# AndersTrier/reed-solomon-simd

Hardware: AMD Instinct MI355X
Metric: GiB/s (original+recovery) encode & decode, device-resident, 1024:1024×1024B (higher is better)
Workload: dtype u8; 1 GPU; encode 1024:1024 x 1024 B, device-resident (rs_encode_device); original_count=1024, recovery_count=1024, parallelism=replicas x1 (independent stripes)

## Files before the change

__graft_entry__.py:

```python
import os
import subprocess
import sys

ROOT = os.path.dirname(os.path.abspath(__file__))
PKG = os.path.join(ROOT, "reed-solomon-simd_amd")
LIB = os.path.join(PKG, "lib", "librs_mi355x.so")
SOURCES = ["csrc/rs_kernels.hip", "csrc/rs_mono.hip", "csrc/rs_repair.hip", "csrc/rs_lane.hip", "csrc/rs_chunks.hip", "csrc/rs_eval.hip", "csrc/rs_update.hip", "csrc/rs_verify.hip", "csrc/rs_codec.cpp", "csrc/gf_tables.cpp"]
HEADERS = ["csrc/rs_device.hpp", "csrc/rs_gf.hpp", "csrc/gf_tables.hpp"]
INCLUDES = {"csrc/rs_repair.hip": ["csrc/rs_mono.hip"], "csrc/rs_verify.hip": ["csrc/rs_mono.hip"]}
HIPCC = os.environ.get("HIPCC", "/opt/rocm/bin/hipcc")
FLAGS = ["--offload-arch=gfx950", "-O3", "-std=c++17", "-fPIC", "-Wall"]
SOURCE_FLAGS = {"csrc/rs_mono.hip": ["-mllvm", "-amdgpu-kernarg-preload-count=14"]}


def _obj(src):
    return os.path.join(PKG, "build", os.path.basename(src) + ".o")


def _stale(target, deps):
    if not os.path.exists(target):
        return True
    t = os.path.getmtime(target)
    return any(os.path.getmtime(d) > t for d in deps)


def build(force: bool = False) -> None:
    os.makedirs(os.path.join(PKG, "lib"), exist_ok=True)
    os.makedirs(os.path.join(PKG, "build"), exist_ok=True)
    hdrs = [os.path.join(PKG, h) for h in HEADERS] + [os.path.join(ROOT, "include", "rs_mi355x.h")]
    procs = []
    for src in SOURCES:
        path = os.path.join(PKG, src)
        deps = [path] + hdrs + [os.path.join(PKG, i) for i in INCLUDES.get(src, [])]
        if force or _stale(_obj(src), deps):
            procs.append(subprocess.Popen([HIPCC] + FLAGS + SOURCE_FLAGS.get(src, []) + ["-c", path, "-o", _obj(src)],
                                          cwd=PKG))
    for p in procs:
        if p.wait() != 0:
            raise RuntimeError(f"hipcc failed: {p.args}")
    objs = [_obj(s) for s in SOURCES]
    if force or procs or _stale(LIB, objs):
        subprocess.run([HIPCC, "--offload-arch=gfx950", "-shared", "-fPIC", "-o", LIB] + objs, check=True)
    ob_src = os.path.join(ROOT, "tools", "object_bench.cpp")
    ob = os.path.join(PKG, "lib", "rs_object_bench")
    if force or _stale(ob, [ob_src, LIB, os.path.join(ROOT, "include", "rs_mi355x.h")]):
        subprocess.run(["g++", "-O2", "-std=c++17", "-I", os.path.join(ROOT, "include"), ob_src, "-o", ob,
                        "-L", os.path.join(PKG, "lib"), "-lrs_mi355x", "-Wl,-rpath,$ORIGIN"], check=True)
    subprocess.run(["make", "-s", "-C", os.path.join(ROOT, "oracle")], check=True)
    sys.path.insert(0, PKG)
    import reed_solomon_simd


def smoke() -> None:
    import numpy as np
    import torch

    sys.path.insert(0, PKG)
    sys.path.insert(0, os.path.join(ROOT, "tests"))
    import oracle_lib as O
    import reed_solomon_simd as rs

# ... 25 lines not shown
```

reed-solomon-simd_amd/csrc/rs_mono.hip:

```cpp
#include <hip/hip_runtime.h>

#include <cstdio>
#include <type_traits>

#include "rs_device.hpp"
#include "rs_gf.hpp"

namespace rs {
namespace {

#ifdef RS_MONO_STAMPS
__device__ uint64_t g_mono_stamps[4096][24];
#ifdef RS_MONO_STAMP_WAIT
#define RS_MSTAMP_WAIT() asm volatile("s_waitcnt vmcnt(0) lgkmcnt(0)" ::: "memory")
#else
#define RS_MSTAMP_WAIT() asm volatile("" ::: "memory")
#endif
#define RS_MSTAMP(i)                                                                                 \
    do {                                                                                             \
        RS_MSTAMP_WAIT();                                                                            \
        if (threadIdx.x == blockDim.x - 64 && blockIdx.x + blockIdx.y * gridDim.x < 4096) g_mono_stamps[blockIdx.x + blockIdx.y * gridDim.x][i] = __builtin_amdgcn_s_memrealtime(); \
    } while (0)
#else
#define RS_MSTAMP(i)
#endif


struct Map {
    int reg[3];
    int lane[6];
    int wave[4];
};
enum : int { kOpLayer = 1, kOpXpose = 2, kOpRemap = 3 };
struct Op {
    int kind, bit, rs, ls;
};
constexpr int kMaxOps = 64;
struct Seq {
    int count = 0;
    Op ops[kMaxOps] = {};
    Map maps[kMaxOps + 1] = {};
};

constexpr int find_reg(const Map &m, int LR, int x) {
    for (int s = 0; s < LR; ++s)
        if (m.reg[s] == x) return s;
    return -1;
}
constexpr int find_lane(const Map &m, int x) {
    for (int j = 0; j < 6; ++j)
        if (m.lane[j] == x) return j;
    return -1;
}
constexpr int next_use(const int *bits, int nb, int from, int x) {
    for (int t = from; t < nb; ++t)
        if (bits[t] == x) return t;
    return 1 << 20;
}
constexpr void push(Seq &s, Op op, const Map &after) {
// ... 177 lines not shown
constexpr int pair_of(int i, int s) { return (i & ((1 << s) - 1)) | ((i >> (s + 1)) << s); }

__device__ __forceinline__ void load_tab(const uint32_t *img, int L, int x, uint32_t row, uint32_t (&t)[20]) {
    const uint32_t n = 1u << L;
    const uint32_t slot = n - (n >> x) + (row >> (x + 1));
#ifdef RS_MONO_FAKE_TABS
    for (int q = 0; q < 20; ++q) t[q] = slot * 0x01010101u + q;
    return;
#endif
    const uint4 *p = reinterpret_cast<const uint4 *>(img) + slot * 5u;
#pragma unroll
    for (int q = 0; q < 5; ++q) {
        const uint4 v = p[q];
        t[4 * q] = v.x, t[4 * q + 1] = v.y, t[4 * q + 2] = v.z, t[4 * q + 3] = v.w;
    }
}

struct GlobalTabs {
    const uint32_t *img;
    template <int L, int LR, typename S, int I, int PH>
    __device__ __forceinline__ void get(int x, uint32_t row, uint32_t (&t)[20]) const {
        load_tab(img, L, x, row, t);
    }
};


#ifndef RS_MONO_SPARE_BARRIERS
#define RS_MONO_SPARE_BARRIERS 0
#endif

template <int L, int LR, int SP = 0, int E = 4>
struct Stage {
    static constexpr bool SPLIT = Plan<L, LR, SP>::SPLIT;
    static constexpr int FLO = Plan<L, LR, SP>::FLO;
    static constexpr int TW = Fmt<E>::kTW;
    static constexpr uint32_t PC = Fmt<E>::kPC;
    static constexpr bool kBasis = E == 2 && RS_MONO_BASIS;
    static constexpr uint32_t LPC = kBasis ? 2 : PC;
    template <typename AT>
    static __device__ __forceinline__ void put(uint32_t *region, uint32_t q, const uint4 &v, AT at) {
        if constexpr (kBasis) {
            const uint32_t p0 = (q >> 1) * PC + (q & 1u) * 2u;
            uint4 a, b;
            basis2_expand(v, a, b);
            reinterpret_cast<uint4 *>(region)[at(p0)] = a;
            reinterpret_cast<uint4 *>(region)[at(p0 + 1)] = b;
        } else {
            reinterpret_cast<uint4 *>(region)[at(q)] = v;
        }
    }
    static constexpr int SW = 20;
    static constexpr uint32_t SPC = SW / 4;
    static constexpr bool kGray = E == 2;
    static __device__ __forceinline__ uint32_t sg(uint32_t g) { return kGray ? g ^ ((g >> 1) & 15u) : g; }
    static __device__ __forceinline__ uint32_t sq(uint32_t t, uint32_t k) {
        if constexpr (!kGray) return t;
        const uint32_t y = (1u << k) - t;
        const uint32_t mask = y <= 1u ? 0u : (1u << (31 - __builtin_clz(y - 1u))) - 1u;
        return t ^ (((t & mask) >> 1) & 15u);
    }
    template <typename F>
    static __device__ __forceinline__ uint32_t at(uint32_t q, F f) {
        const uint32_t t = q / PC;
        return f(t) * SPC + (q - t * PC);
    }
    static __device__ __forceinline__ uint32_t at1(uint32_t q) {
        return at(q, [](uint32_t t) { return sq(t, uint32_t(IW - B0)); });
    }
    static __device__ __forceinline__ uint32_t at0(uint32_t q) { return at(q, [](uint32_t t) { return sg(t); }); }
    static __device__ __forceinline__ uint32_t atS(uint32_t q) {
        return at(q, [](uint32_t t) {
            if (t < kShI) return sq(t, uint32_t(L - IW));
            if (t < kShI + kShF) return kShI + sq(t - kShI, uint32_t(L - FLO));
            return t;
        });
    }
    static constexpr int IW = LR + 6, WB = L - IW - (SPLIT ? 1 : 0);
    static constexpr uint32_t n = 1u << L, W = 1u << IW;
    static constexpr int NB3 = WB > 0 ? FLO : L;
#ifndef RS_MONO_B0_MIN_L
#define RS_MONO_B0_MIN_L 11
#endif
    static constexpr int B0 = L >= RS_MONO_B0_MIN_L ? 1 : 0;
    static constexpr uint32_t kPriv = B0 ? (W >> 1) : W - 1;
    static constexpr uint32_t kUp = (W >> B0) - 1;
    static constexpr uint32_t kP3 = (W >> B0) - (W >> NB3);
    static constexpr uint32_t kL0 = W >> 1;
    static constexpr uint32_t kShI = WB > 0 ? (n >> IW) - 1 : 0;
    static constexpr uint32_t kShF = WB > 0 ? (n >> FLO) - 1 : 0;
    static constexpr uint32_t kShared = kShI + kShF;
    static constexpr uint32_t kWaves = 1u << (L - LR - 6);
    static constexpr uint32_t plane_words = (E == 4 ? 2 : 1) * n;
    static constexpr uint32_t words = plane_words + (kShared + kWaves * kPriv) * SW;
#ifdef RS_MONO_ENC_DERIVE3
    static constexpr bool kDerive3 = true;
#else
    static constexpr bool kDerive3 = false;
#endif
    static constexpr uint32_t kD = kDerive3 ? NB3 : 0;
    static constexpr uint32_t words_enc = words + kD * SW;
    static constexpr bool kPlane2 = RS_MONO_SPARE_BARRIERS && WB > 0 && (words_enc + plane_words) * 4 <= 160 * 1024;
    static constexpr uint32_t words_enc2 = words_enc + (kPlane2 ? plane_words : 0);
    static constexpr uint32_t words_dec = words + n;
    static constexpr uint32_t words_split = words_dec + (SPLIT ? plane_words : 0);
    static_assert(L > 11 || (words_enc2 * 4 <= 160 * 1024 && words_split * 4 <= 160 * 1024), "column kernel: LDS per workgroup");
};

template <int L, int LR, int SPLIT = 0, int E = 4>
struct LdsTabs {
    using G = Stage<L, LR, SPLIT, E>;
    const uint32_t *priv, *shared, *img_i, *img_f;
    template <int, int, typename S, int I, int PH>
    __device__ __forceinline__ void get(int x, uint32_t row, uint32_t (&t)[Fmt<E>::kTW]) const {
#ifdef RS_MONO_FAKE_TABS
        const uint32_t *fb = tab<0, 0, S, I, PH>(x, row);
        for (int q = 0; q < G::TW; ++q) t[q] = q + uint32_t(reinterpret_cast<uintptr_t>(fb));
        return;
#endif
        read(tab<0, 0, S, I, PH>(x, row), t);
    }
    static __device__ __forceinline__ void read(const uint32_t *tb, uint32_t (&t)[Fmt<E>::kTW]) {
        const uint4 *p = reinterpret_cast<const uint4 *>(tb);
#pragma unroll
        for (int q = 0; q < int(G::PC); ++q) {
            const uint4 v = p[q];
            t[4 * q] = v.x, t[4 * q + 1] = v.y, t[4 * q + 2] = v.z, t[4 * q + 3] = v.w;
        }
    }
    template <int, int, typename S, int I, int PH>
    __device__ __forceinline__ const uint32_t *tab(int x, uint32_t row) const {
        uint32_t slot;
        const uint32_t *base;
        if constexpr ((PH == 1 || PH == 3) && G::B0 == 1 && S::v.ops[I].bit == 0) {
            slot = G::sg((row & (G::W - 1)) >> 1);
            base = priv;
        } else if constexpr (PH == 1 || PH == 3) {
            slot = (G::W >> G::B0) - (G::W >> x) + G::sg((row & (G::W - 1)) >> (x + 1));
            base = priv;
        } else if constexpr (PH == 2) {
            slot = (G::n >> G::IW) - (G::n >> x) + G::sg(row >> (x + 1));
            base = shared;
        } else {
            slot = G::kShI + (G::n >> G::FLO) - (G::n >> x) + G::sg(row >> (x + 1));
// ... 1018 lines not shown
        walsh_lane<J, J>(x, lane);
    });
    walsh_reg<WB>(x);
    static_for<WB, 6>([&](auto jc) {
        constexpr int J = decltype(jc)::value;
        walsh_lane<J, J + 1>(x, lane);
    });
    RS_MSTAMP(20);
    eval_remap<L, false>(x, buf, lane, wave);
    static_for<6 - WB, 6>([&](auto jc) {
        constexpr int J = decltype(jc)::value;
        walsh_lane<J, J + WB + 1>(x, lane);
    });
    x[0] = walsh_fold(x[0]);
    x[1] = walsh_fold(x[1]);
    reinterpret_cast<uint2 *>(rinfo)[threadIdx.x] =
        uint2{x[0] | ((rbits & 1u) ? 0u : 0x10000u), x[1] | ((rbits & 2u) ? 0u : 0x10000u)};
    asm volatile("s_waitcnt lgkmcnt(0)" ::: "memory");
}

template <int L>
__device__ __forceinline__ void col_eval_poly(const MonoCore &A, uint32_t ebits, uint32_t rbits, const uint32_t &lwv,
                                              uint32_t *buf, uint32_t *rinfo) {
    if constexpr (kEvalRemap<L>) {
        col_eval_poly_remap<L>(A, ebits, rbits, lwv, buf, rinfo);
        return;
    }
    const uint32_t i0 = 2 * threadIdx.x;
    uint32_t x[2];
    static_for<0, 2>([&](auto kc) {
        constexpr int k = decltype(kc)::value;
        const uint32_t e = (ebits >> k) & 1u, i = i0 + k;
        x[k] = A.low_rate ? (i < A.end ? (e ? 0u : 65534u) : 0u) : e;
    });
    col_walsh<L, 0, 19>(x, buf);
    RS_MSTAMP(14);
    const uint32_t lw[2] = {lwv & 0xFFFFu, lwv >> 16};
    static_for<0, 2>([&](auto kc) {
        constexpr int k = decltype(kc)::value;
        const uint32_t p = x[k] * lw[k];
        uint32_t f = ev_add(p & 0xFFFFu, p >> 16);
        if (A.low_rate && i0 + k == 0) f = ev_add(f, A.lw0);
        x[k] = f;
    });
    col_walsh<L, kWalshRounds<L>, 20>(x, buf);
    reinterpret_cast<uint2 *>(rinfo)[threadIdx.x] =
        uint2{x[0] | ((rbits & 1u) ? 0u : 0x10000u), x[1] | ((rbits & 2u) ? 0u : 0x10000u)};
    asm volatile("s_waitcnt lgkmcnt(0)" ::: "memory");
}

template <int L, int LR, int SPLIT, int E>
__device__ __forceinline__ uint4 priv_piece(const uint32_t *img, uint32_t wave, uint32_t q) {
    using G = Stage<L, LR, SPLIT, E>;
    const uint32_t t = q / G::LPC, piece = q - t * G::LPC;
    const uint32_t y = (G::W >> G::B0) - t;
    const int b = G::IW - int(32 - __builtin_clz(y - 1));
    const uint32_t local = t - ((G::W >> G::B0) - (G::W >> b));
    const uint32_t slot = G::n - (G::n >> b) + wave * (G::W >> (b + 1)) + local;
    return reinterpret_cast<const uint4 *>(img)[slot * G::LPC + piece];
}
template <int L, int LR, int SPLIT, int E>
__device__ __forceinline__ uint4 l0_piece(const uint32_t *img, uint32_t wave, uint32_t q) {
    using G = Stage<L, LR, SPLIT, E>;
    return reinterpret_cast<const uint4 *>(img)[wave * G::kL0 * G::LPC + q];
}
template <int L, int LR, int SPLIT, int E>
__device__ __forceinline__ const uint4 *shared_piece_ptr(const uint32_t *img_i, const uint32_t *img_f, uint32_t q) {
    using G = Stage<L, LR, SPLIT, E>;
    const uint32_t t = q / G::LPC, piece = q - t * G::LPC;
    const uint32_t slot = t < G::kShI ? G::n - (G::n >> G::IW) + t : G::n - (G::n >> G::FLO) + (t - G::kShI);
    return reinterpret_cast<const uint4 *>(t < G::kShI ? img_i : img_f) + slot * G::LPC + piece;
}
template <int L, int LR, int SPLIT, int E>
__device__ __forceinline__ const uint4 *d_piece_ptr(const uint32_t *img_d, uint32_t q) {
    using G = Stage<L, LR, SPLIT, E>;
    static_assert(!G::kBasis, "D tables: full-table images");
    const uint32_t b = q / G::PC, piece = q - b * G::PC;
    return reinterpret_cast<const uint4 *>(img_d) + (G::n - (G::n >> b)) * G::PC + piece;
}
__device__ __forceinline__ uint4 ld_piece(const uint4 *p) {
    typedef uint32_t v4u __attribute__((ext_vector_type(4)));
    const v4u v = *reinterpret_cast<const v4u *>(p);
    return uint4{v.x, v.y, v.z, v.w};
}
__device__ __forceinline__ uint32_t clamp_piece(uint32_t q, uint32_t count) { return q < count ? q : count - 1u; }
template <int L, int LR, int SPLIT, int E>
__device__ __forceinline__ uint32_t priv_layer(uint32_t t) {
    using G = Stage<L, LR, SPLIT, E>;
    const uint32_t y = (G::W >> G::B0) - t;
    return uint32_t(G::IW - int(32 - __builtin_clz(y - 1)));
}

#ifndef RS_MONO_LDS_PF
#define RS_MONO_LDS_PF 2
#endif

constexpr int mono_pk(int mode, bool staged, bool split) {
#ifndef RS_MONO_NO_FLOW
#ifndef RS_MONO_ENC_NO_FLOW
    const bool flow = staged;
#else
    const bool flow = staged && mode == kMonoDecode;
#endif
#else
    const bool flow = false;
#endif
    return (split ? 1 : 0) | (flow ? 2 : 0);
}

template <typename T>
using gptr = __attribute__((address_space(1))) T *;
template <typename T>
__device__ __forceinline__ gptr<T> as_global(T *p) {
    return (gptr<T>)p;
}

template <int MODE, bool STAGED>
using MonoArgT = std::conditional_t<MODE == kMonoDecode && STAGED, MonoArgs, MonoCore>;
template <int MODE, bool STAGED, bool MASKS>
using MonoArgM = std::conditional_t<MASKS, MonoMaskArgs, MonoArgT<MODE, STAGED>>;

template <int L, int LR, int MODE, bool STAGED, bool BATCH, bool SPLIT, int E, bool MASKS = false, bool TWO = false,
          bool VERIFY = false, bool PRE = false, typename KA = MonoArgM<MODE, STAGED, MASKS>>
__device__ __forceinline__ void mono_body(const KA &K, [[maybe_unused]] const MonoLead *lead = nullptr) {
    static_assert(!PRE || (STAGED && !SPLIT && !MASKS && !TWO && !VERIFY &&
                           (MODE == kMonoEncodeHigh || MODE == kMonoEncodeLow)),
                  "preloaded arguments: the staged single-chunk encode");
    static_assert(!VERIFY || (STAGED && !MASKS && !TWO && (MODE == kMonoEncodeHigh || MODE == kMonoEncodeLow)),
                  "verify: the staged single-chunk encode");
    static_assert(!TWO || MODE == kMonoDecode || (!MASKS && MODE == kMonoHalfFDec), "second destination: decodes");
    static_assert(!MASKS || (MODE == kMonoDecode && STAGED && BATCH && !SPLIT),
                  "per-stripe patterns: the staged batch decode, plain plan");
    MonoCore A;
    uint32_t ew[4] = {0, 0, 0, 0}, rw[4] = {0, 0, 0, 0};
    uint32_t skip_stripe = 0;
    if constexpr (PRE) {
        A.packs = lead->packs;
        A.packs_per_xcd = lead->packs_per_xcd;
        A.nsrc = 1;
        A.src[0] = RowMap{lead->src, lead->src_stride, lead->src_begin, lead->src_end};
        A.src[1] = A.src[0];
        A.dst = K.dst;
        A.img = lead->img;
// ... 99 lines not shown
    const uint32_t b = blockIdx.x;
    const uint32_t pk = (b & 7u) * A.packs_per_xcd + (b >> 3);
    if (pk >= A.packs) return;
    StripeBases sb = BATCH ? stripe_bases(A, blockIdx.y) : StripeBases{A.src[0].base, A.src[1].base,
                                                                             const_cast<uint8_t *>(A.dst.base)};
    const PackIO io = E == 4 && MODE != kMonoQuadEnc ? pack_io(A.fmt, pk) : pack_io2(A.fmt, pk);
    Dst2 d2;
    if constexpr (TWO) {
        d2.m = K.dst2;
        d2.base = const_cast<uint8_t *>(K.dst2.base) + (BATCH ? uint64_t(blockIdx.y) * K.dst2_bstride : 0);
    }
    VerifyPre<LR> vp;
    if constexpr (VERIFY) {
        vp.flags = K.flags + (BATCH ? uint64_t(blockIdx.y) * K.flag_bstride : 0);
        vp.sel = K.sel;
    }
    const uint32_t lane = threadIdx.x & 63u;
    const uint32_t wave = __builtin_amdgcn_readfirstlane(threadIdx.x >> 6);
    constexpr bool HALF_I = MODE == kMonoHalfIEnc || MODE == kMonoHalfIDec;
    constexpr bool HALF_F = MODE == kMonoHalfFEnc || MODE == kMonoHalfFDec;
    uint32_t ii = A.ifft_img, fi = A.fft_img, hh = 0;
    if constexpr (HALF_I) {
        hh = A.half0 + blockIdx.y;
        ii += hh * A.ifft_img_step;
        fi = ii;
    } else if constexpr (HALF_F) {
        hh = A.out_half + blockIdx.y;
        fi += hh * A.fft_img_step;
        ii = fi;
    }
    const uint32_t *img_i = A.img + uint64_t(ii) * A.img_words;
    const uint32_t *img_f = A.img + uint64_t(fi) * A.img_words;
    const uint32_t *img_d = A.img + uint64_t(ii ^ fi) * A.img_words;
    C c;
    if constexpr (STAGED) {
      auto staged = [&](auto bytes_c) {
        constexpr int kBytesIO = decltype(bytes_c)::value;
            constexpr bool DEC = MODE == kMonoDecode;
            constexpr bool HSC = MODE == kMonoHalfIDec, HFD = MODE == kMonoHalfFDec;
            constexpr bool QUAD = MODE == kMonoQuadEnc;
            const PackIO io_w = E == 4 ? pack_io(ShardFormat{}, pk) : pack_io2(ShardFormat{}, pk);
            uint32_t *shared = lds + G::plane_words;
            constexpr bool kDerive3 = !DEC && G::kDerive3;
            constexpr uint32_t kSh = kDerive3 ? G::kShared + G::kD : G::kShared;
            uint32_t *priv = shared + kSh * G::SW + wave * G::kPriv * G::SW;
            uint32_t *rinfo = lds + G::words;
            constexpr uint32_t PC = G::PC;
            constexpr uint32_t LPC = G::LPC;
            static_assert(!(G::kBasis && kDerive3), "derived phase-3 tables: full-table images");
            constexpr int KP1 = (LPC * G::kUp + 63) / 64;
            constexpr int KP0 = G::B0 ? (LPC * G::kL0 + 63) / 64 : 1;
            constexpr int KP3 = G::kP3 ? (LPC * G::kP3 + 63) / 64 : 1;
            constexpr int KSH = kSh ? (LPC * kSh + T - 1) / T : 1;
            RS_MSTAMP(0);
            uint32_t ebits = 0, rbits = 0, lwv = 0;
            if constexpr (MASKS) {
                lwv = reinterpret_cast<const uint32_t *>(A.lw_fold)[kEvalRemap<L> ? eval_t_pair<L>(lane, wave)
                                                                                 : threadIdx.x];
                asm volatile("" ::: "memory");
                asm volatile("" : "+s"(ew[0]), "+s"(ew[1]), "+s"(ew[2]), "+s"(ew[3]), "+s"(rw[0]), "+s"(rw[1]),
                             "+s"(rw[2]), "+s"(rw[3]), "+s"(skip_stripe));
                if (skip_stripe) return;
            }
            bool live = true;
            if constexpr (DEC) {
                static_assert(!STAGED || (1u << G::IW) / 32 == 4, "a wave's phase-1 rows: its 4 bitmap words");
                live = (rw[0] | rw[1] | rw[2] | rw[3]) != 0;
            }
            bool out_wave = true;
            if constexpr (SPLIT) out_wave = (wave >> (L - 1 - G::IW)) == A.out_half;
#ifndef RS_MONO_NO_REUSE
            const bool same3 = ii == fi;
            const bool reuse3 = live && (same3 || kDerive3);
#else
            const bool same3 = ii == fi;
            const bool reuse3 = HALF_F;
#endif

            if constexpr (DEC) {
                const uint32_t g = lane >> 4, sh = (2u * lane) & 31u;
                const uint32_t e0 = ew[0], e1 = ew[1], e2 = ew[2], e3 = ew[3], r0 = rw[0], r1 = rw[1], r2 = rw[2], r3 = rw[3];
                ebits = (g == 0 ? e0 : g == 1 ? e1 : g == 2 ? e2 : e3) >> sh;
                rbits = (g == 0 ? r0 : g == 1 ? r1 : g == 2 ? r2 : r3) >> sh;
                if constexpr (!MASKS) {
                    lwv = reinterpret_cast<const uint32_t *>(A.lw_fold)[kEvalRemap<L> ? eval_t_pair<L>(lane, wave)
                                                                                     : threadIdx.x];
                    asm volatile("" ::: "memory");
                }
            }
#ifndef RS_MONO_DEC_LOAD_ALL
            const bool skip = DEC && !live;
#else
            const bool skip = false;
#endif
            uint32_t w[2 << LR] = {};
            uint32_t okm = 0;
            auto issue_rows = [&](auto bytes) {
                issue_col<L, LR, PK, E, decltype(bytes)::value>(A, HALF_I ? hh : 0u, io, sb, w, okm, lane, wave, live);
            };
            uint32_t w2[2 << LR] = {};
            uint32_t okm2 = 0;
            uint32_t wq[4 << LR] = {};
            uint32_t okmq = 0;
            constexpr uint32_t QW = 1u << G::IW;
            constexpr int KQ = QUAD ? int((4 * QW + 63) / 64) : 1;
            uint4 vq[2][KQ];
            uint32_t *const qtab = lds + G::words_enc + wave * 2u * QW * kQuad0Slot;
            auto issue_quad_tabs = [&]() {
                if constexpr (QUAD) {
                    constexpr uint64_t kImg2 = uint64_t((2u << L) - 1u) * 16u;
                    static_for<0, 2>([&](auto fc) {
                        constexpr int f = decltype(fc)::value;
                        const uint4 *src = reinterpret_cast<const uint4 *>(A.lut + (f ? fi : ii) * kImg2) +
                                           uint64_t(wave) * QW * 4u;
                        static_for<0, KQ>([&](auto kc) {
                            const uint32_t q = lane + 64u * decltype(kc)::value;
                            vq[f][kc] = ld_piece(src + (q < 4 * QW ? q : 4 * QW - 1));
                        });
                    });
                }
            };
            auto write_quad_tabs = [&]() {
                if constexpr (QUAD)
                    static_for<0, 2>([&](auto fc) {
                        constexpr int f = decltype(fc)::value;
                        static_for<0, KQ>([&](auto kc) {
                            const uint32_t q = lane + 64u * decltype(kc)::value;
                            if (q < 4 * QW)
                                reinterpret_cast<uint4 *>(qtab + f * QW * kQuad0Slot + (q >> 2) * kQuad0Slot)[q & 3u] =
                                    vq[f][kc];
                        });
                    });
            };
            uint4 v0[KP0], v1[KP1], vs[KSH];
            auto issue_priv = [&]() {
#ifndef RS_MONO_SKIP_STAGE
                if constexpr (G::B0)
                    static_for<0, KP0>([&](auto kc) {
                        const uint32_t q = clamp_piece(lane + 64u * decltype(kc)::value, LPC * G::kL0);
                        v0[kc] = l0_piece<L, LR, PK, E>(img_i, wave, live ? q : q % LPC);
                    });
                static_for<0, KP1>([&](auto kc) {
                    const uint32_t q = clamp_piece(lane + 64u * decltype(kc)::value, LPC * G::kUp);
                    v1[kc] = priv_piece<L, LR, PK, E>(img_i, wave, live ? q : q % LPC);
                });
#endif
            };
            auto issue_shared = [&]() {
#ifndef RS_MONO_SKIP_STAGE
                if constexpr (kSh > 0)
                    static_for<0, KSH>([&](auto kc) {
                        const uint32_t q = clamp_piece(threadIdx.x + T * decltype(kc)::value, LPC * kSh);
                        if constexpr (kSh == G::kShared) {
                            vs[kc] = ld_piece(shared_piece_ptr<L, LR, PK, E>(img_i, img_f, q));
                        } else {
                            const uint4 *src = q < PC * G::kShared ? shared_piece_ptr<L, LR, PK, E>(img_i, img_f, q)
                                                                   : d_piece_ptr<L, LR, PK, E>(img_d, q - PC * G::kShared);
                            vs[kc] = ld_piece(src);
                        }
                    });
#endif
            };
#ifndef RS_MONO_DEC_ORDER
#define RS_MONO_DEC_ORDER 1
#endif
            constexpr int kOrder = RS_MONO_DEC_ORDER;
            constexpr bool kShFirst = kOrder != 2, kPrivFirst = kOrder == 1, kRowsFirst = kOrder != 4;
            const uint32_t *ri = A.rowinfo;
            auto eval = [&]() {
#ifndef RS_MONO_SKIP_EVAL
                col_eval_poly<L>(A, ebits, rbits, lwv, plane, rinfo);
#else
                rinfo[2 * threadIdx.x] = ebits & 1u ? 0x10000u : lwv & 0xFFFFu;
                rinfo[2 * threadIdx.x + 1] = ebits & 2u ? 0x10000u : lwv >> 16;
                __syncthreads();
#endif
            };
            using kIO = std::integral_constant<int, kBytesIO>;
            if constexpr (HALF_F) {
                issue_col<L, LR, PK, E, 0, true>(A, 0, io_w, sb, w, okm, lane, wave, !(A.zero_halves & 1u));
                issue_col<L, LR, PK, E, 0, true>(A, 1, io_w, sb, w2, okm2, lane, wave, !(A.zero_halves & 2u));
                issue_priv();
                issue_shared();
            } else if constexpr (!DEC) {
                if constexpr (VERIFY) verify_select<L, LR, PK>(A, vp, lane, wave);
                if constexpr (QUAD) issue_quad<L, LR, PK>(A, io, sb, wq, okmq, lane, wave);
                else issue_rows(kIO{});
                issue_priv();
                issue_shared();
                issue_quad_tabs();
                if constexpr (VERIFY) verify_issue<L, LR, PK, E>(A, io, sb, vp, lane, wave);
                if constexpr (PRE) {
                    gptr<const uint8_t> bd = as_global(A.dst.base);
                    gptr<uint8_t> sd = as_global(sb.dst);
                    uint64_t std_ = A.dst.stride;
                    uint32_t rbd = A.dst.row_begin, red = A.dst.row_end;
                    asm volatile("" : "+s"(bd), "+s"(sd), "+s"(std_), "+s"(rbd), "+s"(red));
                    A.dst = RowMap{(const uint8_t *)bd, std_, rbd, red};
                    sb.dst = (uint8_t *)sd;
                }
            } else {
                if constexpr (kShFirst) issue_shared();
                RS_MSTAMP(16);
                if (skip) {
                    RS_MSTAMP(18);
                    eval();
                } else {
                    if constexpr (kRowsFirst) issue_rows(kIO{});
                    RS_MSTAMP(17);
                    if constexpr (kPrivFirst) issue_priv();
                    RS_MSTAMP(18);
                    eval();
                }
                ri = rinfo;
                RS_MSTAMP(2);
            }
            ScaleTabs<L, LR, E> st;
            if constexpr (DEC) {
                if constexpr (!kRowsFirst)
                    if (!skip) issue_rows(kIO{});
                scale_issue<L, LR, PK, E>(A, ri, st, lane, wave, !skip);
                if constexpr (!kShFirst) issue_shared();
                if constexpr (!kPrivFirst)
                    if (!skip) issue_priv();
            }
            if constexpr (HSC) scale_issue<L, LR, PK, E>(A, A.rowinfo + (hh << L), st, lane, wave, true);
            RS_MSTAMP(13);
            const LdsTabs<L, LR, PK, E> ts_lds{priv, shared, img_i, img_f};
            constexpr bool kPreAddr = RS_MONO_PRE_ADDR && LR == 1 && L <= 10;
            const auto ts = [&]() {
                if constexpr (kPreAddr) return LdsTabsPre<L, LR, PK, E, !HALF_F, !HALF_I>(ts_lds, lds, lane, wave);
                else return ts_lds;
            }();
            auto write1 = [&]() {
#ifndef RS_MONO_SKIP_STAGE
                static_for<0, KP1>([&](auto kc) {
                    const uint32_t q = lane + 64u * decltype(kc)::value;
                    if (q < LPC * G::kUp) G::put(priv, q, v1[kc], [](uint32_t p) { return G::at1(p); });
                });
#endif
            };
#ifndef RS_MONO_SKIP_STAGE
            if (!skip) {
                if constexpr (G::B0 && !HALF_F)
                    static_for<0, KP0>([&](auto kc) {
                        const uint32_t q = lane + 64u * decltype(kc)::value;
                        if (q < LPC * G::kL0) G::put(priv, q, v0[kc], [](uint32_t p) { return G::at0(p); });
                    });
                else
                    write1();
            }
#ifdef RS_MONO_HALF_RACE_PROBE
            if constexpr (HALF_F) {
                for (uint32_t q = threadIdx.x; q < kSh * G::SW / 4; q += T)
                    reinterpret_cast<uint4 *>(shared)[q] = uint4{0xEEEEEEEEu, 0xEEEEEEEEu, 0xEEEEEEEEu, 0xEEEEEEEEu};
                __syncthreads();
                if (wave != 0)
                    for (int k = 0; k < 8; ++k) __builtin_amdgcn_s_sleep(127);
            }
#endif
            static_for<0, KSH>([&](auto kc) {
                const uint32_t q = threadIdx.x + T * decltype(kc)::value;
                if (q < LPC * kSh) G::put(shared, q, vs[kc], [](uint32_t p) { return G::atS(p); });
            });
            write_quad_tabs();
#endif
            C cb;
            if constexpr (HALF_F) {
                finish_col<L, LR, false>(w, okm, &st, c, lane, io_w);
                finish_col<L, LR, false>(w2, okm2, &st, cb, lane, io_w);
            } else if constexpr (QUAD) {
                finish_quad<L, LR>(wq, okmq, c, lane, io);
                quad_layer0<L, LR, SeqOf<L, LR, false, PK>, 0, false>(c, qtab, lane, wave);
            } else {
                finish_col<L, LR, DEC || HSC>(w, okm, &st, c, lane, io);
            }
            RS_MSTAMP(1);
            uint4 v3[KP3];
            auto issue3 = [&]() {
                if (reuse3) return;
                if constexpr (G::kP3 > 0)
                static_for<0, KP3>([&](auto kc) {
                    const uint32_t q = lane + 64u * decltype(kc)::value;
                    const uint32_t qc = clamp_piece(q, LPC * G::kP3);
                    v3[kc] = priv_piece<L, LR, PK, E>(img_f, wave, out_wave ? qc : qc % LPC);
                });
            };
            auto write3 = [&]() {
                if (reuse3) {
                    if constexpr (kDerive3) {
                        if (same3) return;
                        uint4 x[KP3];
                        static_for<0, KP3>([&](auto kc) {
                            const uint32_t q = lane + 64u * decltype(kc)::value;
                            if (q < PC * G::kP3) {
                                const uint32_t t = q / PC, piece = q - t * PC;
                                const uint4 v = reinterpret_cast<const uint4 *>(priv)[G::at1(q)];
                                const uint4 d = reinterpret_cast<const uint4 *>(shared)[(G::kShared + priv_layer<L, LR, PK, E>(t)) * G::SPC + piece];
                                x[kc] = uint4{v.x ^ d.x, v.y ^ d.y, v.z ^ d.z, v.w ^ d.w};
                            }
                        });
                        static_for<0, KP3>([&](auto kc) {
                            const uint32_t q = lane + 64u * decltype(kc)::value;
                            if (q < PC * G::kP3) reinterpret_cast<uint4 *>(priv)[G::at1(q)] = x[kc];
                        });
                    }
                    return;
                }
                static_for<0, KP3>([&](auto kc) {
                    const uint32_t q = lane + 64u * decltype(kc)::value;
                    if (q < LPC * G::kP3) G::put(priv, q, v3[kc], [](uint32_t p) { return G::at1(p); });
                });
            };
            uint4 v4[KP0];
            auto issue4 = [&](bool need) {
                if constexpr (G::B0)
                    static_for<0, KP0>([&](auto kc) {
                        const uint32_t q = lane + 64u * decltype(kc)::value;
                        const uint32_t qc = clamp_piece(q, LPC * G::kL0);
                        v4[kc] = l0_piece<L, LR, PK, E>(img_f, wave, need ? qc : qc % LPC);
                    });
            };
            auto write4 = [&]() {
                if constexpr (G::B0)
                    static_for<0, KP0>([&](auto kc) {
                        const uint32_t q = lane + 64u * decltype(kc)::value;
                        if (q < LPC * G::kL0) G::put(priv, q, v4[kc], [](uint32_t p) { return G::at0(p); });
                    });
            };
            constexpr bool kPreReveal = (DEC || HFD) && E == 2 && kQuadGather;
            RevealTabs<LR> rt;
            auto pre3 = [&](bool alive) {
                return [&, alive]() {
                    write3();
                    (void)alive;
                    if constexpr (kPreReveal)
                        if (alive) reveal_issue<L, LR, PK, TWO>(A, ri, rt, lane, wave, HFD ? hh << L : 0u, d2);
                };
            };
            if constexpr (SPLIT) {
                constexpr uint32_t kHalfWords = (G::n / 2) / 32;
                uint32_t half_any = 0;
                const uint32_t h = wave >> (L - 1 - G::IW);
                for (uint32_t k = 0; k < kHalfWords; ++k) half_any |= K.received[h * kHalfWords + k];
                run_seq<L, LR, false, RS_MONO_LDS_PF, G::B0 ? 1 : -1, PK>(ts, c, plane, lane, wave, issue3,
                                                                             half_any != 0, live, write1);
                RS_MSTAMP(5);
                using SF = SeqOf<L, LR, true, PK>;
                constexpr int NLF = num_layers(SF::v);
                const bool out = out_wave;
                const bool alive = out && wave_stores<L, LR, PK, TWO>(A, wave, 0, d2);
                constexpr uint32_t kTopI = (G::n >> G::IW) - 2, kTopF = G::kShI + (G::n >> G::FLO) - 2;
                split_top<L, LR>(c, plane, lds + G::words_dec, shared + kTopI * G::SW, shared + kTopF * G::SW, lane, wave,
                                 A.out_half, ii == 0, fi == 0);
                RS_MSTAMP(6);
                issue4(alive);
                run_seq<L, LR, true, RS_MONO_LDS_PF, G::B0 ? NLF - 1 : -1, PK>(ts, c, plane, lane, wave, pre3(alive),
                                                                                  alive, out, write4);
                if (!alive) return;
// ... 562 lines not shown
```

Measured before the change: 272.5 GiB/s.

## Stage twiddle tables into LDS via global_load_lds DMA instead of register staging

Adds a direct global-to-LDS load path (global_load_lds_dwordx4 with M0 set per instruction) for the private, layer-0 and shared twiddle-table staging in the monolithic kernel. It is enabled by default when prefetch is on and the basis/derive paths are off. Source indices are computed by inverting the swizzled LDS layout, and index math moves into a new StageMap header. The aim is to skip the VGPR round trip and the explicit ds_write stores, cutting register pressure and instructions. In exchange it adds inline asm, M0 juggling and vmcnt waits, which can serialise against other outstanding global loads.

```diff
diff --git a/__graft_entry__.py b/__graft_entry__.py
--- a/__graft_entry__.py
+++ b/__graft_entry__.py
@@ -6,7 +6,7 @@
 PKG = os.path.join(ROOT, "reed-solomon-simd_amd")
 LIB = os.path.join(PKG, "lib", "librs_mi355x.so")
 SOURCES = ["csrc/rs_kernels.hip", "csrc/rs_mono.hip", "csrc/rs_repair.hip", "csrc/rs_lane.hip", "csrc/rs_chunks.hip", "csrc/rs_eval.hip", "csrc/rs_update.hip", "csrc/rs_verify.hip", "csrc/rs_codec.cpp", "csrc/gf_tables.cpp"]
-HEADERS = ["csrc/rs_device.hpp", "csrc/rs_gf.hpp", "csrc/gf_tables.hpp"]
+HEADERS = ["csrc/rs_device.hpp", "csrc/rs_gf.hpp", "csrc/rs_stage_map.hpp", "csrc/gf_tables.hpp"]
 INCLUDES = {"csrc/rs_repair.hip": ["csrc/rs_mono.hip"], "csrc/rs_verify.hip": ["csrc/rs_mono.hip"]}
 HIPCC = os.environ.get("HIPCC", "/opt/rocm/bin/hipcc")
 FLAGS = ["--offload-arch=gfx950", "-O3", "-std=c++17", "-fPIC", "-Wall"]
diff --git a/reed-solomon-simd_amd/csrc/rs_mono.hip b/reed-solomon-simd_amd/csrc/rs_mono.hip
--- a/reed-solomon-simd_amd/csrc/rs_mono.hip
+++ b/reed-solomon-simd_amd/csrc/rs_mono.hip
@@ -5,6 +5,7 @@
 
 #include "rs_device.hpp"
 #include "rs_gf.hpp"
+#include "rs_stage_map.hpp"
 
 namespace rs {
 namespace {
@@ -288,29 +289,11 @@
     static constexpr int SW = 20;
     static constexpr uint32_t SPC = SW / 4;
     static constexpr bool kGray = E == 2;
-    static __device__ __forceinline__ uint32_t sg(uint32_t g) { return kGray ? g ^ ((g >> 1) & 15u) : g; }
-    static __device__ __forceinline__ uint32_t sq(uint32_t t, uint32_t k) {
-        if constexpr (!kGray) return t;
-        const uint32_t y = (1u << k) - t;
-        const uint32_t mask = y <= 1u ? 0u : (1u << (31 - __builtin_clz(y - 1u))) - 1u;
-        return t ^ (((t & mask) >> 1) & 15u);
-    }
-    template <typename F>
-    static __device__ __forceinline__ uint32_t at(uint32_t q, F f) {
-        const uint32_t t = q / PC;
-        return f(t) * SPC + (q - t * PC);
-    }
-    static __device__ __forceinline__ uint32_t at1(uint32_t q) {
-        return at(q, [](uint32_t t) { return sq(t, uint32_t(IW - B0)); });
-    }
-    static __device__ __forceinline__ uint32_t at0(uint32_t q) { return at(q, [](uint32_t t) { return sg(t); }); }
-    static __device__ __forceinline__ uint32_t atS(uint32_t q) {
-        return at(q, [](uint32_t t) {
-            if (t < kShI) return sq(t, uint32_t(L - IW));
-            if (t < kShI + kShF) return kShI + sq(t - kShI, uint32_t(L - FLO));
-            return t;
-        });
-    }
+    static __device__ __forceinline__ uint32_t sg(uint32_t g) { return SM::sg(g); }
+    static __device__ __forceinline__ uint32_t sq(uint32_t t, uint32_t k) { return SM::sq(t, k); }
+    static __device__ __forceinline__ uint32_t at1(uint32_t q) { return SM::at1(q); }
+    static __device__ __forceinline__ uint32_t at0(uint32_t q) { return SM::at0(q); }
+    static __device__ __forceinline__ uint32_t atS(uint32_t q) { return SM::atS(q); }
     static constexpr int IW = LR + 6, WB = L - IW - (SPLIT ? 1 : 0);
     static constexpr uint32_t n = 1u << L, W = 1u << IW;
     static constexpr int NB3 = WB > 0 ? FLO : L;
@@ -318,6 +301,7 @@
 #define RS_MONO_B0_MIN_L 11
 #endif
     static constexpr int B0 = L >= RS_MONO_B0_MIN_L ? 1 : 0;
+    using SM = StageMap<L, LR + 6, FLO, B0, E>;
     static constexpr uint32_t kPriv = B0 ? (W >> 1) : W - 1;
     static constexpr uint32_t kUp = (W >> B0) - 1;
     static constexpr uint32_t kP3 = (W >> B0) - (W >> NB3);
@@ -325,6 +309,9 @@
     static constexpr uint32_t kShI = WB > 0 ? (n >> IW) - 1 : 0;
     static constexpr uint32_t kShF = WB > 0 ? (n >> FLO) - 1 : 0;
     static constexpr uint32_t kShared = kShI + kShF;
+    static_assert(SM::PC == PC && SM::SPC == SPC && SM::kUp == kUp && SM::kP3 == kP3 && SM::kL0 == kL0 &&
+                      SM::kPriv == kPriv && SM::kShI == kShI && SM::kShF == kShF,
+                  "rs_stage_map.hpp: the same regions");
     static constexpr uint32_t kWaves = 1u << (L - LR - 6);
     static constexpr uint32_t plane_words = (E == 4 ? 2 : 1) * n;
     static constexpr uint32_t words = plane_words + (kShared + kWaves * kPriv) * SW;
@@ -1449,17 +1436,12 @@
 template <int L, int LR, int SPLIT, int E>
 __device__ __forceinline__ uint4 priv_piece(const uint32_t *img, uint32_t wave, uint32_t q) {
     using G = Stage<L, LR, SPLIT, E>;
-    const uint32_t t = q / G::LPC, piece = q - t * G::LPC;
-    const uint32_t y = (G::W >> G::B0) - t;
-    const int b = G::IW - int(32 - __builtin_clz(y - 1));
-    const uint32_t local = t - ((G::W >> G::B0) - (G::W >> b));
-    const uint32_t slot = G::n - (G::n >> b) + wave * (G::W >> (b + 1)) + local;
-    return reinterpret_cast<const uint4 *>(img)[slot * G::LPC + piece];
+    return reinterpret_cast<const uint4 *>(img)[G::SM::priv_index(wave, q, G::LPC)];
 }
 template <int L, int LR, int SPLIT, int E>
 __device__ __forceinline__ uint4 l0_piece(const uint32_t *img, uint32_t wave, uint32_t q) {
     using G = Stage<L, LR, SPLIT, E>;
-    return reinterpret_cast<const uint4 *>(img)[wave * G::kL0 * G::LPC + q];
+    return reinterpret_cast<const uint4 *>(img)[G::SM::l0_index(wave, q, G::LPC)];
 }
 template <int L, int LR, int SPLIT, int E>
 __device__ __forceinline__ const uint4 *shared_piece_ptr(const uint32_t *img_i, const uint32_t *img_f, uint32_t q) {
@@ -1483,9 +1465,80 @@
 __device__ __forceinline__ uint32_t clamp_piece(uint32_t q, uint32_t count) { return q < count ? q : count - 1u; }
 template <int L, int LR, int SPLIT, int E>
 __device__ __forceinline__ uint32_t priv_layer(uint32_t t) {
-    using G = Stage<L, LR, SPLIT, E>;
-    const uint32_t y = (G::W >> G::B0) - t;
-    return uint32_t(G::IW - int(32 - __builtin_clz(y - 1)));
+    return Stage<L, LR, SPLIT, E>::SM::priv_layer(t);
+}
+
+#ifndef RS_MONO_LDS_DMA
+#define RS_MONO_LDS_DMA 1
+#endif
+__device__ __forceinline__ uint32_t lds_addr(const uint32_t *p) {
+    return uint32_t(reinterpret_cast<uintptr_t>((const __attribute__((address_space(3))) uint32_t *)p));
+}
+__device__ __forceinline__ void glds16(const uint4 *src, uint32_t lds_dst) {
+    uint32_t keep;
+    asm volatile("s_mov_b32 %0, m0\n\ts_mov_b32 m0, %2\n\ts_nop 0\n\tglobal_load_lds_dwordx4 %1, off\n\ts_mov_b32 m0, %0"
+                 : "=&s"(keep)
+                 : "v"(src), "s"(lds_dst)
+                 : "memory");
+}
+__device__ __forceinline__ void glds16(const uint32_t *base, uint32_t byte_off, uint32_t lds_dst) {
+    uint32_t keep;
+    asm volatile("s_mov_b32 %0, m0\n\ts_mov_b32 m0, %2\n\ts_nop 0\n\tglobal_load_lds_dwordx4 %1, %3\n\ts_mov_b32 m0, %0"
+                 : "=&s"(keep)
+                 : "v"(byte_off), "s"(lds_dst), "s"(base)
+                 : "memory");
+}
+template <int N>
+__device__ __forceinline__ void dma_wait() {
+    static_assert(N >= 0 && N < 64, "vmcnt is a 6-bit counter");
+    asm volatile("s_waitcnt vmcnt(%0)" ::"n"(N) : "memory");
+}
+template <typename SM, uint32_t TABLES, int KIND, int KEEP = 0, size_t NK = 1>
+__device__ __forceinline__ void dma_priv(const uint32_t *img, uint32_t wave, uint32_t lane, uint32_t lds_dst,
+                                         uint32_t (&keep)[NK]) {
+    constexpr uint32_t N = TABLES * SM::SPC;
+    static_assert(TABLES <= SM::kPriv, "inside the wave's region");
+    static_assert(KEEP == 0 || NK == SM::insts(TABLES), "one kept index per instruction");
+    static_for<0, int(SM::insts(TABLES))>([&](auto kc_) {
+        constexpr uint32_t kc = decltype(kc_)::value;
+        const uint32_t p = lane + 64u * kc;
+        uint32_t idx;
+        if constexpr (KEEP == 2) {
+            idx = keep[kc];
+        } else if constexpr (KIND == 0) {
+            const auto s = SM::inv0(p);
+            idx = SM::l0_index(wave, s.t * SM::PC + s.piece);
+        } else {
+            constexpr uint32_t s_lo = 64u * kc / SM::SPC, s_hi = (64u * kc + 63u < N ? 64u * kc + 63u : N - 1u) / SM::SPC;
+            constexpr uint32_t k = SM::kSeq;
+            constexpr uint32_t m_lo = SM::layer_mask(s_lo, k), m_hi = SM::layer_mask(s_hi, k);
+            const uint32_t mask = m_lo == m_hi ? m_lo : SM::layer_mask(p / SM::SPC, k);
+            const auto s = SM::inv1_mask(p, mask);
+            idx = SM::priv_table_mask(wave, s.t, mask) * SM::PC + s.piece;
+        }
+        if constexpr (KEEP != 2) idx *= 16u;
+        if constexpr (KEEP == 1) {
+            asm volatile("" : "+v"(idx));
+            keep[kc] = idx;
+        }
+        if (64u * kc + 63u < N || p < N) glds16(img, idx, lds_dst + 1024u * kc);
+    });
+}
+template <typename SM, uint32_t WAVES>
+__device__ __forceinline__ void dma_shared(const uint32_t *img_i, const uint32_t *img_f, uint32_t wave, uint32_t lane,
+                                           uint32_t lds_dst) {
+    constexpr uint32_t N = SM::kShared * SM::SPC;
+    static_for<0, int((N + 64u * WAVES - 1u) / (64u * WAVES))>([&](auto kc_) {
+        constexpr uint32_t kc = decltype(kc_)::value;
+        const uint32_t blk = wave + WAVES * kc;
+        const uint32_t p = lane + 64u * blk;
+        if (p < N) {
+            const auto s = SM::invS(p);
+            glds16(reinterpret_cast<const uint4 *>(s.t < SM::kShI ? img_i : img_f) + SM::shared_table(s.t) * SM::PC +
+                       s.piece,
+                   lds_dst + 1024u * blk);
+        }
+    });
 }
 
 #ifndef RS_MONO_LDS_PF
@@ -1691,6 +1744,11 @@
             constexpr int KP0 = G::B0 ? (LPC * G::kL0 + 63) / 64 : 1;
             constexpr int KP3 = G::kP3 ? (LPC * G::kP3 + 63) / 64 : 1;
             constexpr int KSH = kSh ? (LPC * kSh + T - 1) / T : 1;
+            constexpr bool kDma = RS_MONO_LDS_DMA && PRE && !G::kBasis && !kDerive3;
+            using SM = typename G::SM;
+            [[maybe_unused]] const uint32_t lds_priv = lds_addr(priv), lds_shared = lds_addr(shared);
+            constexpr bool kKeep3 = kDma && !G::B0 && G::kP3 == G::kUp;
+            [[maybe_unused]] uint32_t didx[kKeep3 ? SM::insts(G::kUp) : 1];
             RS_MSTAMP(0);
             uint32_t ebits = 0, rbits = 0, lwv = 0;
             if constexpr (MASKS) {
@@ -1772,22 +1830,34 @@
                     });
             };
             uint4 v0[KP0], v1[KP1], vs[KSH];
+            auto issue_v1 = [&]() {
+#ifndef RS_MONO_SKIP_STAGE
+                static_for<0, KP1>([&](auto kc) {
+                    const uint32_t q = clamp_piece(lane + 64u * decltype(kc)::value, LPC * G::kUp);
+                    v1[kc] = priv_piece<L, LR, PK, E>(img_i, wave, live ? q : q % LPC);
+                });
+#endif
+            };
             auto issue_priv = [&]() {
 #ifndef RS_MONO_SKIP_STAGE
+                if constexpr (kDma) {
+                    if constexpr (G::B0) dma_priv<SM, G::kL0, 0>(img_i, wave, lane, lds_priv, didx);
+                    else dma_priv<SM, G::kUp, 1, kKeep3 ? 1 : 0>(img_i, wave, lane, lds_priv, didx);
+                    return;
+                }
                 if constexpr (G::B0)
                     static_for<0, KP0>([&](auto kc) {
                         const uint32_t q = clamp_piece(lane + 64u * decltype(kc)::value, LPC * G::kL0);
                         v0[kc] = l0_piece<L, LR, PK, E>(img_i, wave, live ? q : q % LPC);
                     });
-                static_for<0, KP1>([&](auto kc) {
-                    const uint32_t q = clamp_piece(lane + 64u * decltype(kc)::value, LPC * G::kUp);
-                    v1[kc] = priv_piece<L, LR, PK, E>(img_i, wave, live ? q : q % LPC);
-                });
-#endif
+#endif
+                issue_v1();
             };
             auto issue_shared = [&]() {
 #ifndef RS_MONO_SKIP_STAGE
-                if constexpr (kSh > 0)
+                if constexpr (kDma) {
+                    if constexpr (kSh > 0) dma_shared<SM, G::kWaves>(img_i, img_f, wave, lane, lds_shared);
+                } else if constexpr (kSh > 0)
                     static_for<0, KSH>([&](auto kc) {
                         const uint32_t q = clamp_piece(threadIdx.x + T * decltype(kc)::value, LPC * kSh);
                         if constexpr (kSh == G::kShared) {
@@ -1827,6 +1897,7 @@
                 else issue_rows(kIO{});
                 issue_priv();
                 issue_shared();
+                if constexpr (kDma && G::B0) issue_v1();
                 issue_quad_tabs();
                 if constexpr (VERIFY) verify_issue<L, LR, PK, E>(A, io, sb, vp, lane, wave);
                 if constexpr (PRE) {
@@ -1880,7 +1951,8 @@
 #endif
             };
 #ifndef RS_MONO_SKIP_STAGE
-            if (!skip) {
+            if constexpr (kDma) {
+            } else if (!skip) {
                 if constexpr (G::B0 && !HALF_F)
                     static_for<0, KP0>([&](auto kc) {
                         const uint32_t q = lane + 64u * decltype(kc)::value;
@@ -1898,10 +1970,11 @@
                     for (int k = 0; k < 8; ++k) __builtin_amdgcn_s_sleep(127);
             }
 #endif
-            static_for<0, KSH>([&](auto kc) {
-                const uint32_t q = threadIdx.x + T * decltype(kc)::value;
-                if (q < LPC * kSh) G::put(shared, q, vs[kc], [](uint32_t p) { return G::atS(p); });
-            });
+            if constexpr (!kDma)
+                static_for<0, KSH>([&](auto kc) {
+                    const uint32_t q = threadIdx.x + T * decltype(kc)::value;
+                    if (q < LPC * kSh) G::put(shared, q, vs[kc], [](uint32_t p) { return G::atS(p); });
+                });
             write_quad_tabs();
 #endif
             C cb;
@@ -1914,10 +1987,18 @@
             } else {
                 finish_col<L, LR, DEC || HSC>(w, okm, &st, c, lane, io);
             }
+            if constexpr (kDma) dma_wait<G::B0 ? KP1 : 0>();
             RS_MSTAMP(1);
             uint4 v3[KP3];
             auto issue3 = [&]() {
                 if (reuse3) return;
+                if constexpr (kDma) {
+                    if constexpr (G::kP3 > 0) {
+                        asm volatile("s_waitcnt lgkmcnt(0)" ::: "memory");
+                        dma_priv<SM, G::kP3, 1, kKeep3 ? 2 : 0>(img_f, wave, lane, lds_priv, didx);
+                    }
+                    return;
+                }
                 if constexpr (G::kP3 > 0)
                 static_for<0, KP3>([&](auto kc) {
                     const uint32_t q = lane + 64u * decltype(kc)::value;
@@ -1944,6 +2025,10 @@
                             if (q < PC * G::kP3) reinterpret_cast<uint4 *>(priv)[G::at1(q)] = x[kc];
                         });
                     }
+                    return;
+                }
+                if constexpr (kDma) {
+                    dma_wait<G::B0 ? KP0 : 0>();
                     return;
                 }
                 static_for<0, KP3>([&](auto kc) {
diff --git a/reed-solomon-simd_amd/csrc/rs_stage_map.hpp b/reed-solomon-simd_amd/csrc/rs_stage_map.hpp
--- /dev/null
+++ b/reed-solomon-simd_amd/csrc/rs_stage_map.hpp
@@ -0,0 +1,134 @@
+#pragma once
+
+#include <cstdint>
+
+#if defined(__HIPCC__)
+#define RS_SM_FN __host__ __device__ __forceinline__ constexpr
+#else
+#define RS_SM_FN inline constexpr
+#endif
+
+namespace rs {
+
+RS_SM_FN uint32_t sm_log2(uint32_t v) { return 31u - uint32_t(__builtin_clz(v)); }
+
+template <int L, int IW, int FLO, int B0, int E>
+struct StageMap {
+    static_assert(E == 4 || E == 2, "pack format");
+    static constexpr uint32_t PC = E == 4 ? 5 : 4;
+    static constexpr uint32_t SPC = 5;
+    static constexpr bool kGray = E == 2;
+    static constexpr uint32_t n = 1u << L, W = 1u << IW;
+    static constexpr bool kTop = L > IW;
+    static constexpr int NB3 = kTop ? FLO : L;
+    static constexpr uint32_t kUp = (W >> B0) - 1;
+    static constexpr uint32_t kP3 = (W >> B0) - (W >> NB3);
+    static constexpr uint32_t kL0 = W >> 1;
+    static constexpr uint32_t kPriv = B0 ? (W >> 1) : W - 1;
+    static constexpr uint32_t kShI = kTop ? (n >> IW) - 1 : 0;
+    static constexpr uint32_t kShF = kTop ? (n >> FLO) - 1 : 0;
+    static constexpr uint32_t kShared = kShI + kShF;
+    static constexpr uint32_t kImgTabs = n - 1;
+    static constexpr uint32_t kSeq = IW - B0;
+
+    static RS_SM_FN uint32_t sg(uint32_t g) { return kGray ? g ^ ((g >> 1) & 15u) : g; }
+    static RS_SM_FN uint32_t layer_mask(uint32_t t, uint32_t k) {
+        const uint32_t y = (1u << k) - t;
+        return y <= 1u ? 0u : (1u << sm_log2(y - 1u)) - 1u;
+    }
+    static RS_SM_FN uint32_t sq(uint32_t t, uint32_t k) {
+        if constexpr (!kGray) return t;
+        const uint32_t mask = layer_mask(t, k);
+        return t ^ (((t & mask) >> 1) & 15u);
+    }
+    template <typename F>
+    static RS_SM_FN uint32_t at(uint32_t q, F f) {
+        const uint32_t t = q / PC;
+        return f(t) * SPC + (q - t * PC);
+    }
+    static RS_SM_FN uint32_t at1(uint32_t q) {
+        return at(q, [](uint32_t t) { return sq(t, kSeq); });
+    }
+    static RS_SM_FN uint32_t at0(uint32_t q) {
+        return at(q, [](uint32_t t) { return sg(t); });
+    }
+    static RS_SM_FN uint32_t atS(uint32_t q) {
+        return at(q, [](uint32_t t) {
+            if (t < kShI) return sq(t, uint32_t(L - IW));
+            if (t < kShI + kShF) return kShI + sq(t - kShI, uint32_t(L - FLO));
+            return t;
+        });
+    }
+
+    static RS_SM_FN uint32_t gray_fix(uint32_t z) {
+        const uint32_t a = z ^ (z >> 1);
+        return a ^ (a >> 2);
+    }
+    static RS_SM_FN uint32_t sg_inv(uint32_t h) { return kGray ? h ^ gray_fix((h >> 1) & 15u) : h; }
+    static RS_SM_FN uint32_t sq_inv_mask(uint32_t s, uint32_t mask) {
+        if constexpr (!kGray) return s;
+        return s ^ gray_fix(((s & mask) >> 1) & 15u);
+    }
+    static RS_SM_FN uint32_t sq_inv(uint32_t s, uint32_t k) { return sq_inv_mask(s, layer_mask(s, k)); }
+
+    struct Src {
+        uint32_t t, piece;
+        bool real;
+    };
+    template <typename F>
+    static RS_SM_FN Src inv(uint32_t p, F table_at) {
+        const uint32_t s = p / SPC, piece = p - s * SPC;
+        const bool real = piece < PC;
+        return Src{table_at(s), real ? piece : PC - 1u, real};
+    }
+    static RS_SM_FN Src inv1(uint32_t p) {
+        return inv(p, [](uint32_t s) { return sq_inv(s, kSeq); });
+    }
+    static RS_SM_FN Src inv1_mask(uint32_t p, uint32_t mask) {
+        return inv(p, [mask](uint32_t s) { return sq_inv_mask(s, mask); });
+    }
+    static RS_SM_FN Src inv0(uint32_t p) {
+        return inv(p, [](uint32_t s) { return sg_inv(s); });
+    }
+    static RS_SM_FN Src invS(uint32_t p) {
+        return inv(p, [](uint32_t s) {
+            if (s < kShI) return sq_inv(s, uint32_t(L - IW));
+            if (s < kShI + kShF) return kShI + sq_inv(s - kShI, uint32_t(L - FLO));
+            return s;
+        });
+    }
+
+    static RS_SM_FN uint32_t priv_layer(uint32_t t) {
+        const uint32_t y = (W >> B0) - t;
+        return uint32_t(IW - int(32 - __builtin_clz(y - 1)));
+    }
+    static RS_SM_FN uint32_t priv_table(uint32_t wave, uint32_t t, uint32_t b) {
+        const uint32_t local = t - ((W >> B0) - (W >> b));
+        return n - (n >> b) + wave * (W >> (b + 1)) + local;
+    }
+    static RS_SM_FN uint32_t priv_table_mask(uint32_t wave, uint32_t t, uint32_t mask) {
+        return t + (n - (W >> B0)) - (mask + 1u) * (2u * (n / W) - 2u - wave);
+    }
+    static RS_SM_FN uint32_t priv_index(uint32_t wave, uint32_t q, uint32_t LPC = PC) {
+        const uint32_t t = q / LPC, piece = q - t * LPC;
+        return priv_table(wave, t, priv_layer(t)) * LPC + piece;
+    }
+    static RS_SM_FN uint32_t l0_index(uint32_t wave, uint32_t q, uint32_t LPC = PC) {
+        return wave * kL0 * LPC + q;
+    }
+    static RS_SM_FN bool shared_from_fft(uint32_t q, uint32_t LPC = PC) { return q / LPC >= kShI; }
+    static RS_SM_FN uint32_t shared_table(uint32_t t) {
+        return t < kShI ? n - (n >> IW) + t : n - (n >> FLO) + (t - kShI);
+    }
+    static RS_SM_FN uint32_t shared_index(uint32_t q, uint32_t LPC = PC) {
+        const uint32_t t = q / LPC, piece = q - t * LPC;
+        return shared_table(t) * LPC + piece;
+    }
+
+    static constexpr uint32_t insts(uint32_t tables) { return (tables * SPC + 63u) / 64u; }
+};
+
+template <int L, int E>
+using EncodeStageMap = StageMap<L, 7, (L > 7 ? 7 : 0), (L >= 11 ? 1 : 0), E>;
+
+}
```

Result: faster. 278.9 GiB/s (median of 6 runs) (+2.4%).
